# AnyLoc/Revisit-Anything

Measured on AMD Instinct MI355X. Metric: query_images_per_sec, higher is better.
Workload: dtype f32

## Files before the change

revisit-anything_amd/csrc/api.hip:

```cpp
#include <stdarg.h>
#include <stdlib.h>
#include <string.h>

#include <cmath>
#include <mutex>
#include <utility>

#include <initializer_list>

#include "ctx.h"

int segvlad_ctx::fail(int code, const char* fmt, ...) {
  va_list ap;
  va_start(ap, fmt);
  vsnprintf(err, sizeof(err), fmt, ap);
  va_end(ap);
  return code;
}

bool sv_is_device_ptr(const void* p) {
  hipPointerAttribute_t a;
  memset(&a, 0, sizeof(a));
  hipError_t e = hipPointerGetAttributes(&a, p);
  if (e != hipSuccess) {
// ... 133 lines not shown
  if (!c->profiling || c->scope_mute) return;
  t = &c->timers[name];
  if (t->used * 2 >= (int)t->ev.size()) {
    hipEvent_t a = nullptr, b = nullptr;
    (void)hipEventCreate(&a);
    (void)hipEventCreate(&b);
    t->ev.push_back(a);
    t->ev.push_back(b);
  }
  slot = t->used++;
  (void)hipEventRecord(t->ev[2 * slot], c->stream);
}
StageScope::~StageScope() {
  if (t) (void)hipEventRecord(t->ev[2 * slot + 1], ctx->stream);
}

#define CHECK_NO_OPEN_DESCRIBE(what)                                                                                        \
  if (ctx->mask_branch_on_side)                                                                                             \
  return ctx->fail(SEGVLAD_ERR_STATE, what ": a segvlad_describe_begin is open on this context (call segvlad_describe_end first)")

hipError_t sv_max_dyn_lds(const void* fn, size_t bytes) {
  static std::mutex mu;
  static std::map<std::pair<int, const void*>, size_t> done;
  int dev = 0;
  hipError_t e = hipGetDevice(&dev);
  if (e != hipSuccess) return e;
  std::lock_guard<std::mutex> lk(mu);
  auto it = done.find({dev, fn});
  if (it != done.end() && it->second >= bytes) return hipSuccess;
  e = hipFuncSetAttribute(fn, hipFuncAttributeMaxDynamicSharedMemorySize, (int)bytes);
  if (e == hipSuccess) done[{dev, fn}] = bytes;
  return e;
}

extern "C" {

int segvlad_version(void) { return 300; }

int segvlad_create(segvlad_ctx** out, int device_id) {
  if (!out) return SEGVLAD_ERR_ARG;
  *out = nullptr;
  int ndev = 0;
  if (hipGetDeviceCount(&ndev) != hipSuccess || device_id < 0 || device_id >= ndev) return SEGVLAD_ERR_HIP;
  if (hipSetDevice(device_id) != hipSuccess) return SEGVLAD_ERR_HIP;
  segvlad_ctx* c = new (std::nothrow) segvlad_ctx();
  if (!c) return SEGVLAD_ERR_NOMEM;
  c->device = device_id;
  static const char* const env_keys[][2] = {{"SEGVLAD_KNN_FILTER", "knn_filter"},   {"SEGVLAD_F16_CFG", "f16_cfg"},
                                            {"SEGVLAD_F16_GM", "f16_gm"},           {"SEGVLAD_X3_TILE", "x3_tile"},
                                            {"SEGVLAD_X3_GM", "x3_gm"},             {"SEGVLAD_SEARCH_STATS", "search_stats"},
                                            {"SEGVLAD_ASSIGN_NARROW", "assign_narrow"}, {"SEGVLAD_DEBUG_SEARCH", "debug_search"},
                                            {"SEGVLAD_AGG_KPB", "agg_kpb"},
                                            {"SEGVLAD_KNN_HEURISTIC", "knn_heuristic"}, {"SEGVLAD_PCA_PATH", "pca_path"},
                                            {"SEGVLAD_COVER_ROWS", "cover_rows"}};
  for (auto& kv : env_keys)
    if (const char* v = getenv(kv[0])) (void)segvlad_set_option(c, kv[1], v);
#define SV_TAG_P(n) c->n.tag = #n; c->n.fixed = true;
#define SV_TAG_S(n) c->n.tag = #n;
  SV_PERSISTENT_BUFS(SV_TAG_P)
  SV_SCRATCH_BUFS(SV_TAG_S)
#undef SV_TAG_P
#undef SV_TAG_S
  if (const char* v = getenv("SEGVLAD_GUARD")) {
    if (v[0] && v[0] != '0') {
      c->guard = true;
      c->for_each_buf([](DevBuf& b) { b.guard = true; });
    }
  }
  if (const char* v = getenv("SEGVLAD_RCCL_LIB")) snprintf(sv_rccl_lib_override, sizeof(sv_rccl_lib_override), "%s", v);
  if (getenv("SEGVLAD_KNN_FP32")) (void)segvlad_set_option(c, "knn_filter", "fp32");
  if (getenv("SEGVLAD_PCA_FP32")) (void)segvlad_set_option(c, "pca_arith", "fp32");
  c->err[0] = 0;
  *out = c;
  return SEGVLAD_OK;
}

int segvlad_set_option(segvlad_ctx* ctx, const char* key, const char* value) {
  if (!ctx) return SEGVLAD_ERR_ARG;
  if (!key || !value) return ctx->fail(SEGVLAD_ERR_ARG, "set_option: null key/value");
  SvOptions& o = ctx->opt;
  auto as_int = [&](int* dst) -> int {
    char* end = nullptr;
    const long v = strtol(value, &end, 10);
    if (end == value || *end) return ctx->fail(SEGVLAD_ERR_ARG, "set_option(%s): '%s' is not an integer", key, value);
    *dst = (int)v;
    return SEGVLAD_OK;
  };
  if (!strcmp(key, "knn_filter")) {
    if (!strcmp(value, "auto")) o.knn_filter = 0;
    else if (!strcmp(value, "f16")) o.knn_filter = 1;
    else if (!strcmp(value, "bf16x3")) o.knn_filter = 2;
    else if (!strcmp(value, "fp32")) o.knn_filter = 3;
    else return ctx->fail(SEGVLAD_ERR_ARG, "set_option(knn_filter): want auto|f16|bf16x3|fp32, got '%s'", value);
    return SEGVLAD_OK;
  }
  if (!strcmp(key, "pca_arith")) {
    if (!strcmp(value, "auto") || !strcmp(value, "f16x3")) o.pca_fp32 = 0;
    else if (!strcmp(value, "fp32")) o.pca_fp32 = 1;
    else return ctx->fail(SEGVLAD_ERR_ARG, "set_option(pca_arith): want auto|f16x3|fp32, got '%s'", value);
    return SEGVLAD_OK;
  }
  if (!strcmp(key, "pca_path")) {
    if (!strcmp(value, "auto")) o.pca_path = 0;
    else if (!strcmp(value, "planes")) o.pca_path = 1;
    else if (!strcmp(value, "project")) o.pca_path = 2;
    else return ctx->fail(SEGVLAD_ERR_ARG, "set_option(pca_path): want auto|planes|project, got '%s'", value);
    return SEGVLAD_OK;
  }
  auto as_dev = [&](int* dst, std::initializer_list<int> product_values, std::initializer_list<int> probe_values = {}) -> int {
    int v = *dst;
    SV_TRY(as_int(&v));
    bool ok = false;
    for (int a : product_values) ok = ok || a == v;
#ifdef SEGVLAD_ABLATIONS
    for (int a : probe_values) ok = ok || a == v;
#else
    (void)probe_values;
#endif
    if (!ok)
      return ctx->fail(SEGVLAD_ERR_ARG, "set_option(%s=%d): a development switch -- this library holds the default kernels only "
                       "(SEGVLAD_BUILD_ABLATIONS=1 builds lib/libsegvlad_hip_abl.so with the probes of csrc/segvlad_dev.h)", key, v);
    *dst = v;
    return SEGVLAD_OK;
  };
  if (!strcmp(key, "f16_cfg")) return as_dev(&o.f16_cfg, {-1, 250, 300, 62, 63}, {93, 94, 95});
  if (!strcmp(key, "f16_gm")) return as_int(&o.f16_gm);
  if (!strcmp(key, "f16_walk")) return as_int(&o.f16_walk);
  if (!strcmp(key, "f16_deep_cfg")) return as_dev(&o.f16_deep_cfg, {-1, 4, 5});
  if (!strcmp(key, "f16_buf")) return as_dev(&o.f16_buf, {-1, 0});
  if (!strcmp(key, "tnk_gram")) return as_int(&o.tnk_gram);
  if (!strcmp(key, "tnk_fork")) return as_int(&o.tnk_fork);
  if (!strcmp(key, "x3_tile")) return as_int(&o.x3_tile);
  if (!strcmp(key, "x3_gm")) return as_int(&o.x3_gm);
  if (!strcmp(key, "search_stats")) return as_int(&o.search_stats);
  if (!strcmp(key, "knn_heuristic")) return as_int(&o.knn_heuristic);
  if (!strcmp(key, "assign_narrow")) return as_int(&o.assign_narrow);
  if (!strcmp(key, "agg_kpb")) return as_int(&o.agg_kpb);
  if (!strcmp(key, "pj_nw")) return as_int(&o.pj_nw);
  if (!strcmp(key, "pj_f16")) return as_int(&o.pj_f16);
  if (!strcmp(key, "cover_rows")) return as_int(&o.cover_rows);
  if (!strcmp(key, "small_plan")) return as_int(&o.small_plan);
  if (!strcmp(key, "small_tail")) return as_int(&o.small_tail);
  if (!strcmp(key, "small_head")) return as_int(&o.small_head);
  if (!strcmp(key, "batch_l0_f16")) return as_int(&o.batch_l0_f16);
  if (!strcmp(key, "level_carry")) return as_int(&o.level_carry);
  if (!strcmp(key, "f16_persist_wgs")) return as_int(&o.f16_persist_wgs);
  if (!strcmp(key, "debug_small_tail")) return as_int(&o.debug_small_tail);
  if (!strcmp(key, "refine_group")) return as_int(&o.refine_group);
  if (!strcmp(key, "query_group")) return as_int(&o.query_group);
  if (!strcmp(key, "debug_search")) return as_int(&o.debug_search);
  if (!strcmp(key, "debug_fail_search")) return as_int(&o.debug_fail_search);
  if (!strcmp(key, "guard_undersize")) {
    if (!ctx->guard) return ctx->fail(SEGVLAD_ERR_STATE, "set_option(guard_undersize): the context was not created under SEGVLAD_GUARD=1");
    const char* colon = strchr(value, ':');
    bool found = false;
    ctx->for_each_buf([&](DevBuf& b) {
      if (!colon) b.shrink = 0;
      else if (strlen(b.tag) == (size_t)(colon - value) && !strncmp(b.tag, value, (size_t)(colon - value))) {
        b.shrink = atoi(colon + 1);
        found = true;
      }
    });
    if (colon && !found) return ctx->fail(SEGVLAD_ERR_ARG, "set_option(guard_undersize): no buffer named like '%s'", value);
    return SEGVLAD_OK;
  }
  return ctx->fail(SEGVLAD_ERR_ARG, "set_option: unknown key '%s'", key);
}

int segvlad_destroy(segvlad_ctx* ctx) {
  if (!ctx) return SEGVLAD_OK;
  (void)hipSetDevice(ctx->device);
  (void)hipStreamSynchronize(ctx->stream);
  sv_comm_release(ctx);
  if (ctx->side) {
    (void)hipStreamSynchronize(ctx->side);
    (void)hipStreamDestroy(ctx->side);
    (void)hipEventDestroy(ctx->ev_fork);
    (void)hipEventDestroy(ctx->ev_join);
  }
  if (ctx->h_pin) {
    (void)hipHostFree(ctx->h_pin);
    (void)hipEventDestroy(ctx->ev_scalars);
  }
  if (ctx->h_desc) (void)hipHostFree(ctx->h_desc);
  if (ctx->ev_desc) (void)hipEventDestroy(ctx->ev_desc);
  ctx->for_each_buf([](DevBuf& b) { b.release(); });
  for (auto& kv : ctx->timers)
    for (hipEvent_t e : kv.second.ev)
      if (e) (void)hipEventDestroy(e);
  delete ctx;
  return SEGVLAD_OK;
}

// ... 987 lines not shown
```

revisit-anything_amd/csrc/ctx.h:

```cpp
#pragma once
#include <hip/hip_runtime.h>
#include <stdint.h>
#include <stdio.h>
#include <string.h>

#include <map>
#include <string>
#include <vector>

#include "../../include/segvlad.h"

#define SV_HIP(expr)                                                                              \
  do {                                                                                            \
    hipError_t _e = (expr);                                                                       \
    if (_e != hipSuccess) {                                                                       \
      return ctx->fail(SEGVLAD_ERR_HIP, "%s failed: %s (%s:%d)", #expr, hipGetErrorString(_e),    \
                       __FILE__, __LINE__);                                                       \
    }                                                                                             \
  } while (0)

#define SV_TRY(expr)          \
  do {                        \
    int _r = (expr);          \
    if (_r != SEGVLAD_OK) return _r; \
// ... 42 lines not shown
    size_t want = bytes + bytes / 8 + 256;
    hipError_t e = hipMalloc(&p, want);
    if (e != hipSuccess) return e;
    cap = want;
    return hipSuccess;
  }
  hipError_t reserve_guarded(size_t bytes);
  size_t fence_off() const { return fixed ? cap : ((req > (size_t)shrink ? req - (size_t)shrink : 0) + 3) & ~(size_t)3; }
  void release() {
    if (raw) (void)hipFree(raw);
    else if (p) (void)hipFree(p);
    raw = nullptr;
    p = nullptr;
    cap = 0;
    req = 0;
  }
  template <class T>
  T* as() { return reinterpret_cast<T*>(p); }
};

struct StageTimer {
  std::vector<hipEvent_t> ev;
  int used = 0;
  int launches = 0;
};

struct SvOptions {
  int knn_filter = 0;
  int pca_fp32 = 0;
  int f16_cfg = -1;
  int f16_gm = -1;
  int f16_walk = -1;
  int f16_persist_wgs = 32;
  int f16_deep_cfg = -1;
  int f16_buf = -1;
  int tnk_gram = 1;
  int tnk_fork = 1;
  int x3_tile = 0;
  int x3_gm = -1;
  int search_stats = 0;
  int knn_heuristic = 1;
  int assign_narrow = 0;
  int agg_kpb = 4;
  int debug_fail_search = 0;
  int debug_search = 0;
  int debug_small_tail = 0;
  int batch_l0_f16 = 1;
  int level_carry = 1;
  int small_head = 1;
  int small_tail = 1;
  int small_plan = 1;
  int pj_f16 = 1;
  int pj_nw = 8;
  int refine_group = 1;
  int query_group = 0;
  int pca_path = 0;
  int cover_rows = 1;
};

constexpr int SV_F16_KBLOCK = 1024;
inline int sv_f16_kblock(const SvOptions& o, int d) {
  if (o.f16_cfg == 300) return SV_F16_KBLOCK;
  return (o.f16_cfg < 0 && d >= 4096) ? SV_F16_KBLOCK : 0;
}
constexpr int SV_F16_KFLUSH = 64;
int sv_f16_eps_kblock(const SvOptions& o, int d);
inline bool sv_f16_bias_possible(const SvOptions& o, int64_t nq) { return nq > 128 && (o.f16_cfg < 0 || o.f16_cfg == 250 || o.f16_cfg == 300); }
enum class F16Kernel {
  None, BatchDefault, BatchComplement, BatchSmall, BatchUnbiased, BatchUnbiasedSmall, DeepFlush, DeepFlushComplement, DeepBlockedBuf, DeepBlocked,
  DeepBlockedBufComplement, DeepBlockedComplement, DeepUnbiased, OneImage64, OneImage128,
#ifdef SEGVLAD_ABLATIONS
  ProbePhases, ProbeNoEpilogue, ProbeNoEpilogueNoDma,
#endif
};
struct F16Choice {
  F16Kernel kernel;
  const char* why;
};
F16Choice sv_choose_f16_kernel(const SvOptions& o, bool bias_ok, int M, int64_t n_rows, int d, int b_stride, int skip);
inline float sv_f16_c_eps(int d, int kb, float bias_mult) {
  const float acc = kb > 0 ? (2.f * (float)kb + (float)((d + kb - 1) / kb) + 1.f) / 16777216.f : 2.f * (float)d / 16777216.f;
  return 2.5f * (1.f / 1024.f + 1.f / 4194304.f + bias_mult * acc);
}

struct SvSearchStats {
  int64_t levels = 0;
  int64_t filter = 0;
  int64_t n_fallback = 0;
  int64_t cand_max = 0;
  int64_t cand_sum = 0;
  int64_t refine_max = 0;
  int64_t refine_sum = 0;
  int64_t n_queries = 0;
  int64_t n_redo = 0;
  int64_t n_refine2 = 0;
  int64_t grp_groups = 0;
  int64_t grp_union_sum = 0;
  int64_t carry_rows = 0;
};

struct segvlad_ctx {
  int device = 0;
  hipStream_t stream = nullptr;
  hipStream_t side = nullptr;
  hipEvent_t ev_fork = nullptr, ev_join = nullptr;
  uint32_t* h_pin = nullptr;
// ... 281 lines not shown
```

revisit-anything_amd/csrc/project_kernels.hip:

```cpp
#include "ctx.h"

typedef float f32x16 __attribute__((ext_vector_type(16)));
#define MFMA32(a, b, c) __builtin_amdgcn_mfma_f32_32x32x2f32((a), (b), (c), 0, 0, 0)
__device__ __forceinline__ int pj_frag_row(int r, int kk) { return (r & 3) + 8 * (r >> 2) + 4 * kk; }

__global__ __launch_bounds__(1024) void group_plan_kernel(const int32_t* __restrict__ cov_cnt, int B, int K,
                                                          int32_t* __restrict__ rowbase, int32_t* __restrict__ tile_group,
                                                          int max_tiles) {
  __shared__ int32_t part[1024], base[257];
  const int nsl = 1024 / K;
  const int k = threadIdx.x % K, c = threadIdx.x / K;
  const int per = (B + nsl - 1) / nsl, b0 = c * per, b1 = min(B, b0 + per);
  const bool act = c < nsl;
  for (int t = threadIdx.x; t < max_tiles; t += blockDim.x) tile_group[t] = -1;
  int sum = 0;
  if (act)
    for (int b = b0; b < b1; ++b) sum += cov_cnt[(size_t)b * K + k];
  part[threadIdx.x] = act ? sum : 0;
  __syncthreads();
  if ((int)threadIdx.x < K) {
    int run = 0;
    for (int q = 0; q < nsl; ++q) {
      const int v = part[q * K + threadIdx.x];
      part[q * K + threadIdx.x] = run;
// ... 1 lines not shown
    }
    base[threadIdx.x + 1] = (run + 255) & ~255;
  }
  __syncthreads();
  if (threadIdx.x == 0) {
    base[0] = 0;
    for (int q = 0; q < K; ++q) base[q + 1] += base[q];
  }
  __syncthreads();
  if (act) {
    int run = base[k] + part[threadIdx.x];
    for (int b = b0; b < b1; ++b) {
      rowbase[(size_t)b * K + k] = run;
      run += cov_cnt[(size_t)b * K + k];
    }
  }
  __syncthreads();
  if ((int)threadIdx.x < K)
    for (int t = base[threadIdx.x] >> 8; t < (base[threadIdx.x + 1] >> 8) && t < max_tiles; ++t) tile_group[t] = threadIdx.x;
}

int sv_launch_group_plan(segvlad_ctx* ctx, const int32_t* cov_cnt, int B, int K, int32_t* rowbase, int32_t* tile_group,
                         int max_tiles) {
  if (K > 256) return ctx->fail(SEGVLAD_ERR_LIMIT, "group_plan: K=%d > 256", K);
  hipLaunchKernelGGL(group_plan_kernel, dim3(1), dim3(1024), 0, ctx->stream, cov_cnt, B, K, rowbase, tile_group, max_tiles);
  SV_HIP(hipGetLastError());
  return SEGVLAD_OK;
}

__global__ __launch_bounds__(256) void project_consts_kernel(const float* __restrict__ comps, const float* __restrict__ mean,
                                                             int P, int64_t KD, float* __restrict__ wmu) {
  const int p = blockIdx.x;
  const float* w = comps + (size_t)p * KD;
  double acc = 0.0;
  for (int64_t j = threadIdx.x; j < KD; j += 256) acc += (double)w[j] * (double)mean[j];
  __shared__ double red[256];
  red[threadIdx.x] = acc;
  __syncthreads();
  for (int o = 128; o > 0; o >>= 1) {
    if ((int)threadIdx.x < o) red[threadIdx.x] += red[threadIdx.x + o];
    __syncthreads();
  }
  if (threadIdx.x == 0) wmu[p] = (float)red[0];
}

int sv_launch_project_consts(segvlad_ctx* ctx, const float* comps, const float* mean, int P, int64_t KD, float* wmu) {
  hipLaunchKernelGGL(project_consts_kernel, dim3(P), dim3(256), 0, ctx->stream, comps, mean, P, KD, wmu);
  SV_HIP(hipGetLastError());
  return SEGVLAD_OK;
}

constexpr int PJ_T = 32;

template <int NW, bool F16 = false>
__global__ __launch_bounds__(64 * NW) void project_aggregate_kernel(const float* __restrict__ Z, const float* __restrict__ wmu,
                                                                const float* __restrict__ bn, const float* __restrict__ gscale,
                                                                const uint64_t* __restrict__ colmask,
                                                                const int32_t* __restrict__ lab_off,
                                                                const int32_t* __restrict__ rowbase,
                                                                const int32_t* __restrict__ phys,
                                                                const int32_t* __restrict__ seg_off, int N, int K, int P, int SC,
                                                                int maxt, const float* __restrict__ col_scale,
                                                                float* __restrict__ Y, float zscale) {
  extern __shared__ __attribute__((aligned(16))) unsigned char smem[];
  typedef _Float16 f16x8 __attribute__((ext_vector_type(8)));
  static_assert(!F16 || NW == 8, "16-bit tile sums: the 8-wave workgroup");
  const int KS = K + 1 + (K & 1);
  float* ag = reinterpret_cast<float*>(smem);
  constexpr int NC = 32 * NW, NT_ = 64 * NW, C4W = NC / 4;
  float* zt = ag + 64 * KS;
  uint64_t* mk = reinterpret_cast<uint64_t*>(zt + 2 * PJ_T * NC);
  int32_t* tl_k = reinterpret_cast<int32_t*>(mk + 2 * PJ_T);
  int32_t* tl_j = tl_k + maxt;
  int32_t* tl_z = tl_j + maxt;
  int32_t* tl_n = tl_z + maxt;
  int32_t* phl = tl_n + maxt + K + 1;
  uint4* af = reinterpret_cast<uint4*>((reinterpret_cast<uintptr_t>(phl + N) + 15) & ~(uintptr_t)15);
  __shared__ int s_tiles;
  const int b = blockIdx.y, p0 = blockIdx.x * NC;
  const int tid = threadIdx.x, w = tid >> 6, l = tid & 63, i = l & 31, kk = l >> 5;
  const int s0 = seg_off[b], S = seg_off[b + 1] - s0;
  const int SCb = (S + 63) >> 6;
  const int32_t* lo = lab_off + (size_t)b * (K + 1);
  const int pcol = p0 + 32 * w + i;
  int32_t* tl_pre = tl_n + maxt;
  int my_o0 = 0, my_n = 0, my_g0 = 0;
  if (tid < K) {
    my_o0 = lo[tid];
    my_n = lo[tid + 1] - my_o0;
    my_g0 = rowbase[(size_t)b * K + tid];
    tl_pre[tid + 1] = (my_n + PJ_T - 1) / PJ_T;
  }
  for (int j = tid; j < N; j += NT_) phl[j] = phys[(size_t)b * N + j];
  __syncthreads();
  if (tid == 0) {
    int run = 0;
    tl_pre[0] = 0;
    for (int k = 0; k < K; ++k) {
      run += tl_pre[k + 1];
      tl_pre[k + 1] = run;
    }
    s_tiles = run < maxt ? run : maxt;
  }
  __syncthreads();
  if (tid < K) {
    int t = tl_pre[tid];
    for (int j0 = 0; j0 < my_n && t < maxt; j0 += PJ_T, ++t) {
      tl_k[t] = tid;
      tl_j[t] = my_o0 + j0;
      tl_z[t] = my_g0;
      tl_n[t] = min(PJ_T, my_n - j0);
    }
  }
  __syncthreads();
  const int tiles = s_tiles;

  for (int sc = 0; sc < SCb; ++sc) {
    const int Sc = min(64, S - 64 * sc);
    __syncthreads();
    for (int idx = tid; idx < 64 * K; idx += NT_) {
      const int s = idx / K, k = idx - s * K;
      float a = 0.f;
      if (s < Sc) {
        const float nrm = bn[(size_t)(s0 + 64 * sc + s) * K + k];
        a = nrm > 1e-12f ? gscale[s0 + 64 * sc + s] / nrm : 0.f;
      }
      if (F16) ag[k * 64 + s] = a;
      else ag[s * KS + k] = a;
    }
    f32x16 acc[2];
// ... 73 lines not shown
      _Pragma("unroll") for (int ks = 0; ks < 2; ++ks) {                                                        \
        if (ks == 1 && nt_ <= 16) break;                                                                        \
        f16x8 hh, ll;                                                                                           \
        _Pragma("unroll") for (int e = 0; e < 8; ++e) {                                                         \
          const float v = ztc[(size_t)(16 * ks + e) * NC] * zscale;                                             \
          hh[e] = (_Float16)v;                                                                                  \
          ll[e] = (_Float16)(v - (float)hh[e]);                                                                 \
        }                                                                                                       \
        const uint4 a0u = afc[(2 * ks) * 64];                                                                   \
        const f16x8 a0 = __builtin_bit_cast(f16x8, a0u);                                                        \
        if (ks == 0) {                                                                                          \
          f32x16 zero_;                                                                                         \
          _Pragma("unroll") for (int r = 0; r < 16; ++r) zero_[r] = 0.f;                                        \
          ta0 = __builtin_amdgcn_mfma_f32_32x32x16_f16(a0, ll, zero_, 0, 0, 0);                                 \
        } else {                                                                                                \
          ta0 = __builtin_amdgcn_mfma_f32_32x32x16_f16(a0, ll, ta0, 0, 0, 0);                                   \
        }                                                                                                       \
        ta0 = __builtin_amdgcn_mfma_f32_32x32x16_f16(a0, hh, ta0, 0, 0, 0);                                     \
        if (two) {                                                                                              \
          const uint4 a1u = afc[(2 * ks + 1) * 64];                                                             \
          const f16x8 a1 = __builtin_bit_cast(f16x8, a1u);                                                      \
          if (ks == 0) {                                                                                        \
            f32x16 zero_;                                                                                       \
            _Pragma("unroll") for (int r = 0; r < 16; ++r) zero_[r] = 0.f;                                      \
            ta1 = __builtin_amdgcn_mfma_f32_32x32x16_f16(a1, ll, zero_, 0, 0, 0);                               \
          } else {                                                                                              \
            ta1 = __builtin_amdgcn_mfma_f32_32x32x16_f16(a1, ll, ta1, 0, 0, 0);                                 \
          }                                                                                                     \
          ta1 = __builtin_amdgcn_mfma_f32_32x32x16_f16(a1, hh, ta1, 0, 0, 0);                                   \
        }                                                                                                       \
      }                                                                                                         \
       \
      const float* agk = ag + k_ * 64 + 4 * kk;                                                                 \
      _Pragma("unroll") for (int q = 0; q < 4; ++q) {                                                           \
        const float4 w0 = *reinterpret_cast<const float4*>(agk + 8 * q);                                        \
        acc[0][4 * q + 0] = fmaf(w0.x, ta0[4 * q + 0], acc[0][4 * q + 0]);                                      \
        acc[0][4 * q + 1] = fmaf(w0.y, ta0[4 * q + 1], acc[0][4 * q + 1]);                                      \
        acc[0][4 * q + 2] = fmaf(w0.z, ta0[4 * q + 2], acc[0][4 * q + 2]);                                      \
        acc[0][4 * q + 3] = fmaf(w0.w, ta0[4 * q + 3], acc[0][4 * q + 3]);                                      \
        if (two) {                                                                                              \
          const float4 w1 = *reinterpret_cast<const float4*>(agk + 32 + 8 * q);                                 \
          acc[1][4 * q + 0] = fmaf(w1.x, ta1[4 * q + 0], acc[1][4 * q + 0]);                                    \
          acc[1][4 * q + 1] = fmaf(w1.y, ta1[4 * q + 1], acc[1][4 * q + 1]);                                    \
          acc[1][4 * q + 2] = fmaf(w1.z, ta1[4 * q + 2], acc[1][4 * q + 2]);                                    \
          acc[1][4 * q + 3] = fmaf(w1.w, ta1[4 * q + 3], acc[1][4 * q + 3]);                                    \
        }                                                                                                       \
      }                                                                                                         \
    } while (0)
#define SV_PJ_MULX(t_)                                                                                          \
    do {                                                                                                        \
      if constexpr (F16) SV_PJ_MUL16(t_);                                                                       \
      else SV_PJ_MUL(t_);                                                                                       \
    } while (0)
    if (tiles > 0) {
      SV_PJ_FETCH(va, ma, 0);
      SV_PJ_FETCH_F(fa, 0);
      SV_PJ_STASH(va, ma, 0);
      SV_PJ_STASH_F(fa, 0);
    }
    if (tiles > 1) {
      SV_PJ_FETCH(va, ma, 1);
      SV_PJ_FETCH_F(fa, 1);
    }
    __syncthreads();
    for (int t = 0; t < tiles; t += 2) {
      if (t + 2 < tiles) {
        SV_PJ_FETCH(vb, mb, t + 2);
        SV_PJ_FETCH_F(fb, t + 2);
      }
      SV_PJ_MULX(t);
      if (t + 1 < tiles) {
        SV_PJ_STASH(va, ma, 1);
        SV_PJ_STASH_F(fa, 1);
      }
      __syncthreads();
      if (t + 1 >= tiles) break;
      if (t + 3 < tiles) {
        SV_PJ_FETCH(va, ma, t + 3);
        SV_PJ_FETCH_F(fa, t + 3);
      }
      SV_PJ_MULX(t + 1);
      if (t + 2 < tiles) {
        SV_PJ_STASH(vb, mb, 0);
        SV_PJ_STASH_F(fb, 0);
      }
      __syncthreads();
    }
#undef SV_PJ_MULX
#undef SV_PJ_MUL16
#undef SV_PJ_STASH_F
#undef SV_PJ_FETCH_F
#undef SV_PJ_MUL
#undef SV_PJ_STASH
#undef SV_PJ_FETCH
    if (pcol < P) {
      const float cs = col_scale ? col_scale[pcol] : 1.f, mu = wmu[pcol];
#pragma unroll
      for (int mt = 0; mt < 2; ++mt) {
        if (mt == 1 && !two) break;
#pragma unroll
        for (int r = 0; r < 16; ++r) {
          const int s = 32 * mt + pj_frag_row(r, kk);
          if (s < Sc) Y[(size_t)(s0 + 64 * sc + s) * P + pcol] = ((F16 ? acc[mt][r] * (1.f / zscale) : acc[mt][r]) - mu) * cs;
        }
      }
    }
  }
}

int sv_launch_project_aggregate(segvlad_ctx* ctx, const float* Z, const float* wmu, const float* block_norms, const float* gscale,
                                const uint64_t* colmask, const int32_t* lab_off, const int32_t* rowbase, const int32_t* phys,
                                const int32_t* seg_off_dev, int B, int N, int K, int P, int SC, int S_max, const float* col_scale,
                                float* Y, float zscale) {
  if (B <= 0 || S_max <= 0) return SEGVLAD_OK;
  if (P % 4) return ctx->fail(SEGVLAD_ERR_ARG, "project_aggregate: P=%d must be a multiple of 4", P);
  const int maxt = K + (N + PJ_T - 1) / PJ_T;
  const int nw = ctx->opt.pj_nw == 4 ? 4 : 8;
  if (K > 64 * nw) return ctx->fail(SEGVLAD_ERR_LIMIT, "project_aggregate: K=%d clusters need %d threads", K, K);
  const bool f16 = zscale > 0.f && nw == 8 && ctx->opt.pj_f16 != 0;
  const size_t lds = (size_t)64 * (K + 1 + (K & 1)) * 4 + (size_t)2 * PJ_T * 32 * nw * 4 + (size_t)2 * PJ_T * 8 + (size_t)4 * maxt * 4 +
                     (size_t)(K + 1) * 4 + (size_t)N * 4 + (f16 ? 16 + 2 * 256 * 16 : 0);
  if (lds > 160 * 1024)
    return ctx->fail(SEGVLAD_ERR_LIMIT, "project_aggregate: K=%d, N=%d need %zu B of LDS", K, N, lds);
  const void* fn = f16 ? reinterpret_cast<const void*>(project_aggregate_kernel<8, true>)
                       : nw == 8 ? reinterpret_cast<const void*>(project_aggregate_kernel<8>) : reinterpret_cast<const void*>(project_aggregate_kernel<4>);
  if (lds > 64 * 1024) SV_HIP(sv_max_dyn_lds(fn, (size_t)lds));
  const dim3 grid((P + 32 * nw - 1) / (32 * nw), B), block(64 * nw);
  if (f16)
    hipLaunchKernelGGL((project_aggregate_kernel<8, true>), grid, block, lds, ctx->stream, Z, wmu, block_norms, gscale, colmask, lab_off,
                       rowbase, phys, seg_off_dev, N, K, P, SC, maxt, col_scale, Y, zscale);
  else if (nw == 8)
    hipLaunchKernelGGL(project_aggregate_kernel<8>, grid, block, lds, ctx->stream, Z, wmu, block_norms, gscale, colmask, lab_off, rowbase,
                       phys, seg_off_dev, N, K, P, SC, maxt, col_scale, Y, 0.f);
  else
    hipLaunchKernelGGL(project_aggregate_kernel<4>, grid, block, lds, ctx->stream, Z, wmu, block_norms, gscale, colmask, lab_off, rowbase,
                       phys, seg_off_dev, N, K, P, SC, maxt, col_scale, Y, 0.f);
  SV_HIP(hipGetLastError());
  return SEGVLAD_OK;
}
```

revisit-anything_amd/csrc/vlad_kernels.hip:

```cpp
#include <stdio.h>
#include <stdlib.h>

#include "ctx.h"

typedef float f32x16 __attribute__((ext_vector_type(16)));

#define MFMA32(a, b, c) __builtin_amdgcn_mfma_f32_32x32x2f32((a), (b), (c), 0, 0, 0)

template <int CTRL>
__device__ __forceinline__ float dpp_f32(float x) {
  return __int_as_float(__builtin_amdgcn_update_dpp(0, __float_as_int(x), CTRL, 0xf, 0xf, true));
}

__device__ __forceinline__ int frag_row(int r, int kk) { return (r & 3) + 8 * (r >> 2) + 4 * kk; }

__global__ void vocab_norm_kernel(const float* __restrict__ C, int K, int D, float* __restrict__ inv) {
  const int k = blockIdx.x;
  float s = 0.f;
  for (int d = threadIdx.x; d < D; d += blockDim.x) {
    float v = C[(size_t)k * D + d];
    s = fmaf(v, v, s);
  }
  __shared__ float red[256];
  red[threadIdx.x] = s;
// ... 537 lines not shown
  _Pragma("unroll") for (int j = 0; j < 4; ++j) {                                     \
    const int d_ = lr + 8 * j;                                                        \
    float* q = tile + (buf) * (DC * TS) + d_ * TS + ((4 * lq + rot(d_)) & 127);       \
    *reinterpret_cast<float4*>(q) = V[j];                                             \
  }
  SV_LOAD_CHUNK(va, 0)
  SV_PARK_CHUNK(va, 0)
  if (1 < nch) { SV_LOAD_CHUNK(va, 1) }
  __syncthreads();
#define SV_ASSIGN_STEP(c, VNEXT, VFREE)                                               \
  {                                                                                   \
    if ((c) + 2 < nch) { SV_LOAD_CHUNK(VFREE, (c) + 2) }                              \
    assign_wide_chunk<NT>(tile + ((c) & 1) * (DC * TS), bt, Xt, b, N, D, t0, tid, w, l, i, kk, (c), acc, ss);  \
    if ((c) + 1 < nch) { SV_PARK_CHUNK(VNEXT, ((c) + 1) & 1) }                        \
    __syncthreads();                                                                  \
  }
  for (int c = 0; c < nch; c += 2) {
    SV_ASSIGN_STEP(c, va, vb)
    if (c + 1 < nch) SV_ASSIGN_STEP(c + 1, vb, va)
  }
#undef SV_ASSIGN_STEP
#undef SV_LOAD_CHUNK
#undef SV_PARK_CHUNK
  constexpr int KP = NT * 32;
  float* sc = tile;
  ss += __shfl_xor(ss, 32);
  if (kk == 0) ssum[32 * w + i] = ss;
#pragma unroll
  for (int n = 0; n < NT; ++n)
#pragma unroll
    for (int r = 0; r < 16; ++r) sc[(32 * w + frag_row(r, kk)) * (KP + 1) + n * 32 + i] = acc[n][r];
  __syncthreads();
  if (tid < 128 && t0 + tid < N) {
    const float rn = 1.0f / fmaxf(sqrtf(ssum[tid]), 1e-12f);
    float best = -INFINITY, second = -INFINITY;
    int bi = 0;
    for (int k = 0; k < K; ++k) {
      const float sv = sc[tid * (KP + 1) + k];
      if (sv > best) {
        second = best;
        best = sv;
        bi = k;
      } else if (sv > second) {
        second = sv;
      }
    }
    const size_t o = (size_t)b * N + t0 + tid;
    labels[o] = (uint8_t)bi;
    rnorm[o] = rn;
    if (gap) gap[o] = (K > 1) ? (best - second) * rn : INFINITY;
  }
}

int sv_launch_assign(segvlad_ctx* ctx, const float* tokens, int B, int N, float* xt, uint8_t* labels, float* rnorm,
                     float* gap) {
  const int NT = ctx->Kpad / 32;
  dim3 grid((N + 63) / 64, B), block(256);
  const float* bt = ctx->vocab_bt.as<float>();
  if (NT <= 2 && ctx->D % 32 == 0 && !ctx->opt.assign_narrow) {
    const unsigned tiles_total = (unsigned)((N + 127) / 128) * (unsigned)B;
    dim3 gridw((tiles_total + 7) / 8 * 8, 1);
    if (NT == 1)
      hipLaunchKernelGGL(assign_wide_kernel<1>, gridw, block, 0, ctx->stream, tokens, N, ctx->D, ctx->K, bt, xt, labels, rnorm, gap, B);
    else
      hipLaunchKernelGGL(assign_wide_kernel<2>, gridw, block, 0, ctx->stream, tokens, N, ctx->D, ctx->K, bt, xt, labels, rnorm, gap, B);
    SV_HIP(hipGetLastError());
    return SEGVLAD_OK;
  }
  switch (NT) {
    case 1:
      hipLaunchKernelGGL(assign_kernel<1>, grid, block, 0, ctx->stream, tokens, N, ctx->D, ctx->K, bt, xt, labels, rnorm, gap);
      break;
    case 2: {
#ifdef SEGVLAD_ABLATIONS
      const char* ab = getenv("SEGVLAD_ASSIGN_ABL");
      const int a = ab ? atoi(ab) : 0;
      if (a == 1) {
        hipLaunchKernelGGL((assign_kernel<2, 1>), grid, block, 0, ctx->stream, tokens, N, ctx->D, ctx->K, bt, xt, labels, rnorm, gap);
        break;
      } else if (a == 2) {
        hipLaunchKernelGGL((assign_kernel<2, 2>), grid, block, 0, ctx->stream, tokens, N, ctx->D, ctx->K, bt, xt, labels, rnorm, gap);
        break;
      } else if (a == 3) {
        hipLaunchKernelGGL((assign_kernel<2, 3>), grid, block, 0, ctx->stream, tokens, N, ctx->D, ctx->K, bt, xt, labels, rnorm, gap);
        break;
      }
#endif
      hipLaunchKernelGGL(assign_kernel<2>, grid, block, 0, ctx->stream, tokens, N, ctx->D, ctx->K, bt, xt, labels, rnorm, gap);
      break;
    }
    case 4:
      hipLaunchKernelGGL(assign_kernel<4>, grid, block, 0, ctx->stream, tokens, N, ctx->D, ctx->K, bt, xt, labels, rnorm, gap);
      break;
    default:
      return ctx->fail(SEGVLAD_ERR_LIMIT, "K=%d: supported cluster counts are 1..64 and 97..128 (Kpad in {32,64,128})", ctx->K);
  }
  SV_HIP(hipGetLastError());
  return SEGVLAD_OK;
}

__global__ __launch_bounds__(256) void prep_kernel(const uint8_t* __restrict__ labels, const uint64_t* __restrict__ inc,
                                                   const int32_t* __restrict__ seg_off,
                                                   const int64_t* __restrict__ adj_off, const uint8_t* __restrict__ adj,
                                                   int N, int K, int S_max, int SC, uint64_t* __restrict__ colmask,
                                                   float* __restrict__ gscale, int32_t* __restrict__ tok_order,
                                                   int32_t* __restrict__ lab_off, const float* __restrict__ rnorm,
                                                   float* __restrict__ rn_sorted, int stage, int ord_n,
                                                   int32_t* __restrict__ phys, int32_t* __restrict__ cov_cnt, int cover) {
  extern __shared__ __attribute__((aligned(16))) unsigned char smem[];
  const int b = blockIdx.x;
  const int nw = (N + 63) >> 6;
  const int s0 = seg_off[b], S = seg_off[b + 1] - s0;
  uint64_t* inc2 = reinterpret_cast<uint64_t*>(smem);
  uint64_t* lbits = inc2 + (size_t)S_max * nw;
// ... 858 lines not shown
```

Baseline: 8680.

## Add register-staged software pipelining to assign and project-aggregate kernels

Adds new scheduled variants of the assign kernel and the project-aggregate kernel. Both prefetch the next tiles into registers two steps ahead and park them into double-buffered LDS after the MFMA work, so global loads overlap compute. The assign variant can also double-buffer the vocabulary slice. The variants are on by default through a new describe_sched option, and launches now go through hipLaunchKernel with an argument array. This uses more registers and LDS, which may lower occupancy.

```diff
diff --git a/revisit-anything_amd/csrc/api.hip b/revisit-anything_amd/csrc/api.hip
--- a/revisit-anything_amd/csrc/api.hip
+++ b/revisit-anything_amd/csrc/api.hip
@@ -209,7 +209,7 @@
                                             {"SEGVLAD_ASSIGN_NARROW", "assign_narrow"}, {"SEGVLAD_DEBUG_SEARCH", "debug_search"},
                                             {"SEGVLAD_AGG_KPB", "agg_kpb"},
                                             {"SEGVLAD_KNN_HEURISTIC", "knn_heuristic"}, {"SEGVLAD_PCA_PATH", "pca_path"},
-                                            {"SEGVLAD_COVER_ROWS", "cover_rows"}};
+                                            {"SEGVLAD_COVER_ROWS", "cover_rows"},   {"SEGVLAD_DESCRIBE_SCHED", "describe_sched"}};
   for (auto& kv : env_keys)
     if (const char* v = getenv(kv[0])) (void)segvlad_set_option(c, kv[1], v);
 #define SV_TAG_P(n) c->n.tag = #n; c->n.fixed = true;
@@ -296,6 +296,7 @@
   if (!strcmp(key, "pj_nw")) return as_int(&o.pj_nw);
   if (!strcmp(key, "pj_f16")) return as_int(&o.pj_f16);
   if (!strcmp(key, "cover_rows")) return as_int(&o.cover_rows);
+  if (!strcmp(key, "describe_sched")) return as_int(&o.describe_sched);
   if (!strcmp(key, "small_plan")) return as_int(&o.small_plan);
   if (!strcmp(key, "small_tail")) return as_int(&o.small_tail);
   if (!strcmp(key, "small_head")) return as_int(&o.small_head);
diff --git a/revisit-anything_amd/csrc/ctx.h b/revisit-anything_amd/csrc/ctx.h
--- a/revisit-anything_amd/csrc/ctx.h
+++ b/revisit-anything_amd/csrc/ctx.h
@@ -118,6 +118,7 @@
   int small_plan = 1;
   int pj_f16 = 1;
   int pj_nw = 8;
+  int describe_sched = 1;
   int refine_group = 1;
   int query_group = 0;
   int pca_path = 0;
diff --git a/revisit-anything_amd/csrc/project_kernels.hip b/revisit-anything_amd/csrc/project_kernels.hip
--- a/revisit-anything_amd/csrc/project_kernels.hip
+++ b/revisit-anything_amd/csrc/project_kernels.hip
@@ -77,7 +77,7 @@
 
 constexpr int PJ_T = 32;
 
-template <int NW, bool F16 = false>
+template <int NW, bool F16 = false, bool SCHED = false>
 __global__ __launch_bounds__(64 * NW) void project_aggregate_kernel(const float* __restrict__ Z, const float* __restrict__ wmu,
                                                                 const float* __restrict__ bn, const float* __restrict__ gscale,
                                                                 const uint64_t* __restrict__ colmask,
@@ -100,7 +100,8 @@
   int32_t* tl_z = tl_j + maxt;
   int32_t* tl_n = tl_z + maxt;
   int32_t* phl = tl_n + maxt + K + 1;
-  uint4* af = reinterpret_cast<uint4*>((reinterpret_cast<uintptr_t>(phl + N) + 15) & ~(uintptr_t)15);
+  uint4* af = SCHED ? reinterpret_cast<uint4*>(smem + ((static_cast<size_t>(reinterpret_cast<unsigned char*>(phl + N) - smem) + 15) & ~(size_t)15))
+                    : reinterpret_cast<uint4*>((reinterpret_cast<uintptr_t>(phl + N) + 15) & ~(uintptr_t)15);
   __shared__ int s_tiles;
   const int b = blockIdx.y, p0 = blockIdx.x * NC;
   const int tid = threadIdx.x, w = tid >> 6, l = tid & 63, i = l & 31, kk = l >> 5;
@@ -280,6 +281,75 @@
       if constexpr (F16) SV_PJ_MUL16(t_);                                                                       \
       else SV_PJ_MUL(t_);                                                                                       \
     } while (0)
+#define SV_PJ_FETCH_S(V, KM, M, R, NTV, t_)                                                                      \
+    do {                                                                                                        \
+      const int nt_ = tl_n[t_], j_ = tl_j[t_];                                                                  \
+      const float* src_ = Z + (size_t)tl_z[t_] * P;                                                             \
+      const int32_t* ph_ = phl + j_;                                                                            \
+      NTV = nt_;                                                                                                \
+      KM = 0u;                                                                                                  \
+      _Pragma("unroll") for (int q = 0; q < 4; ++q) {                                                           \
+        const int idx4 = tid + NT_ * q, row = idx4 / C4W, c4 = idx4 % C4W;                                      \
+        const int pr_ = row < nt_ ? ph_[row] : -1;                                                              \
+        const bool ok_ = pr_ >= 0 && p0 + 4 * c4 < P;                                                           \
+        KM |= ok_ ? (1u << q) : 0u;                                                                             \
+        V[q] = *reinterpret_cast<const float4*>(ok_ ? src_ + (size_t)pr_ * P + p0 + 4 * c4 : Z);                \
+      }                                                                                                         \
+      if constexpr (F16) {                                                                                      \
+        const int j0_ = 16 * ((tid >> 7) & 1) + 8 * ((tid & 63) >> 5);                                          \
+        const uint32_t* mrow_ = reinterpret_cast<const uint32_t*>(colmask + ((size_t)b * N + j_) * SC + sc) + ((tid >> 6) & 1); \
+        _Pragma("unroll") for (int e = 0; e < 8; ++e) R[e] = mrow_[(size_t)min(j0_ + e, nt_ - 1) * SC * 2];     \
+      } else {                                                                                                  \
+        M = colmask[((size_t)b * N + j_ + min(tid & (PJ_T - 1), nt_ - 1)) * SC + sc];                           \
+      }                                                                                                         \
+    } while (0)
+#define SV_PJ_STASH_S(V, KM, M, R, NTV, buf_)                                                                    \
+    do {                                                                                                        \
+      _Pragma("unroll") for (int q = 0; q < 4; ++q) {                                                           \
+        const int idx4 = tid + NT_ * q, row = idx4 / C4W, c4 = idx4 % C4W;                                      \
+        *reinterpret_cast<float4*>(zt + (size_t)(buf_) * PJ_T * NC + row * NC + 4 * c4) =                       \
+            ((KM >> q) & 1u) ? V[q] : make_float4(0.f, 0.f, 0.f, 0.f);                                          \
+      }                                                                                                         \
+      if constexpr (F16) {    \
+        const int s5_ = tid & 31, j0_ = 16 * ((tid >> 7) & 1) + 8 * ((tid & 63) >> 5);                          \
+        uint32_t d_[4];                                                                                         \
+        _Pragma("unroll") for (int q = 0; q < 4; ++q) {                                                         \
+          const bool b0_ = j0_ + 2 * q < NTV && ((R[2 * q] >> s5_) & 1u);                                       \
+          const bool b1_ = j0_ + 2 * q + 1 < NTV && ((R[2 * q + 1] >> s5_) & 1u);                               \
+          d_[q] = (b0_ ? 0x3C00u : 0u) | (b1_ ? 0x3C000000u : 0u);                                              \
+        }                                                                                                       \
+        if (tid < 256) af[(buf_) * 256 + tid] = make_uint4(d_[0], d_[1], d_[2], d_[3]);                         \
+      } else {                                                                                                  \
+        if (tid < PJ_T) mk[(buf_) * PJ_T + tid] = tid < NTV ? M : 0ull;                                         \
+      }                                                                                                         \
+    } while (0)
+#define SV_PJ_STEP(t_, VN, KN, MN, RN, NN, VF, KF, MF, RF, NF, MORE)                                             \
+    {                                                                                                           \
+      if (MORE || (t_) + 2 < tiles) SV_PJ_FETCH_S(VF, KF, MF, RF, NF, (t_) + 2);                                \
+      SV_PJ_MULX(t_);                                                                                           \
+      if (MORE || (t_) + 1 < tiles) SV_PJ_STASH_S(VN, KN, MN, RN, NN, ((t_) + 1) & 1);                          \
+      __syncthreads();                                                                                          \
+    }
+    if constexpr (SCHED) {
+      unsigned ka = 0u, kb = 0u;
+      int na = 0, nb = 0;
+      uint32_t ra[8], rb[8];
+      if (tiles > 0) {
+        SV_PJ_FETCH_S(va, ka, ma, ra, na, 0);
+        SV_PJ_STASH_S(va, ka, ma, ra, na, 0);
+      }
+      if (tiles > 1) SV_PJ_FETCH_S(va, ka, ma, ra, na, 1);
+      __syncthreads();
+      int t = 0;
+      for (; t + 3 < tiles; t += 2) {
+        SV_PJ_STEP(t, va, ka, ma, ra, na, vb, kb, mb, rb, nb, true)
+        SV_PJ_STEP(t + 1, vb, kb, mb, rb, nb, va, ka, ma, ra, na, true)
+      }
+      for (; t < tiles; t += 2) {
+        SV_PJ_STEP(t, va, ka, ma, ra, na, vb, kb, mb, rb, nb, false)
+        if (t + 1 < tiles) SV_PJ_STEP(t + 1, vb, kb, mb, rb, nb, va, ka, ma, ra, na, false)
+      }
+    } else {
     if (tiles > 0) {
       SV_PJ_FETCH(va, ma, 0);
       SV_PJ_FETCH_F(fa, 0);
@@ -314,6 +384,10 @@
       }
       __syncthreads();
     }
+    }
+#undef SV_PJ_STEP
+#undef SV_PJ_STASH_S
+#undef SV_PJ_FETCH_S
 #undef SV_PJ_MULX
 #undef SV_PJ_MUL16
 #undef SV_PJ_STASH_F
@@ -333,6 +407,7 @@
         }
       }
     }
+    if constexpr (SCHED) __builtin_amdgcn_s_waitcnt(0x0F70);
   }
 }
 
@@ -350,19 +425,20 @@
                      (size_t)(K + 1) * 4 + (size_t)N * 4 + (f16 ? 16 + 2 * 256 * 16 : 0);
   if (lds > 160 * 1024)
     return ctx->fail(SEGVLAD_ERR_LIMIT, "project_aggregate: K=%d, N=%d need %zu B of LDS", K, N, lds);
-  const void* fn = f16 ? reinterpret_cast<const void*>(project_aggregate_kernel<8, true>)
-                       : nw == 8 ? reinterpret_cast<const void*>(project_aggregate_kernel<8>) : reinterpret_cast<const void*>(project_aggregate_kernel<4>);
+  const bool sched = ctx->opt.describe_sched != 0;
+  const void* fn = sched ? (f16       ? reinterpret_cast<const void*>(project_aggregate_kernel<8, true, true>)
+                            : nw == 8 ? reinterpret_cast<const void*>(project_aggregate_kernel<8, false, true>)
+                                      : reinterpret_cast<const void*>(project_aggregate_kernel<4, false, true>))
+                         : (f16       ? reinterpret_cast<const void*>(project_aggregate_kernel<8, true>)
+                            : nw == 8 ? reinterpret_cast<const void*>(project_aggregate_kernel<8>)
+                                      : reinterpret_cast<const void*>(project_aggregate_kernel<4>));
   if (lds > 64 * 1024) SV_HIP(sv_max_dyn_lds(fn, (size_t)lds));
   const dim3 grid((P + 32 * nw - 1) / (32 * nw), B), block(64 * nw);
-  if (f16)
-    hipLaunchKernelGGL((project_aggregate_kernel<8, true>), grid, block, lds, ctx->stream, Z, wmu, block_norms, gscale, colmask, lab_off,
-                       rowbase, phys, seg_off_dev, N, K, P, SC, maxt, col_scale, Y, zscale);
-  else if (nw == 8)
-    hipLaunchKernelGGL(project_aggregate_kernel<8>, grid, block, lds, ctx->stream, Z, wmu, block_norms, gscale, colmask, lab_off, rowbase,
-                       phys, seg_off_dev, N, K, P, SC, maxt, col_scale, Y, 0.f);
-  else
-    hipLaunchKernelGGL(project_aggregate_kernel<4>, grid, block, lds, ctx->stream, Z, wmu, block_norms, gscale, colmask, lab_off, rowbase,
-                       phys, seg_off_dev, N, K, P, SC, maxt, col_scale, Y, 0.f);
+  const float zs = f16 ? zscale : 0.f;
+  void* args[] = {(void*)&Z,    (void*)&wmu,     (void*)&block_norms, (void*)&gscale, (void*)&colmask, (void*)&lab_off, (void*)&rowbase,
+                  (void*)&phys, (void*)&seg_off_dev, (void*)&N,       (void*)&K,      (void*)&P,       (void*)&SC,      (void*)&maxt,
+                  (void*)&col_scale, (void*)&Y,  (void*)&zs};
+  SV_HIP(hipLaunchKernel(fn, grid, block, args, lds, ctx->stream));
   SV_HIP(hipGetLastError());
   return SEGVLAD_OK;
 }
diff --git a/revisit-anything_amd/csrc/vlad_kernels.hip b/revisit-anything_amd/csrc/vlad_kernels.hip
--- a/revisit-anything_amd/csrc/vlad_kernels.hip
+++ b/revisit-anything_amd/csrc/vlad_kernels.hip
@@ -613,6 +613,143 @@
   }
 }
 
+template <int NT, int NB>
+__global__ __launch_bounds__(256, NB == 1 ? 4 : 3) void assign_sched_kernel(const float* __restrict__ T, int N, int D, int K,
+                                                           const float* __restrict__ bt, float* __restrict__ Xt,
+                                                           uint8_t* __restrict__ labels, float* __restrict__ rnorm,
+                                                           float* __restrict__ gap, int B) {
+  constexpr int DC = 32, TS = 128, BL = (DC / 2) * NT * 64;
+  constexpr int KP = NT * 32;
+  auto rot = [](int d) { return 8 * (d >> 2) + 32 * (d & 1); };
+  __shared__ __attribute__((aligned(16))) float lds[2 * DC * TS + NB * BL];
+  static_assert(128 * (KP + 1) + 128 <= 2 * DC * TS + NB * BL, "the scores and the squared norms reuse the tiles");
+  float* tile = lds;
+  float* bl = lds + 2 * DC * TS;
+  const int gx = (N + 127) / 128;
+  const int per = (int)((gridDim.x + 7) / 8);
+  const int logical = (int)(blockIdx.x & 7) * per + (int)(blockIdx.x >> 3);
+  if (logical >= gx * B) return;
+  const int b = logical / gx, t0 = (logical - b * gx) * 128;
+  const int tid = threadIdx.x, w = tid >> 6, l = tid & 63, i = l & 31, kk = l >> 5;
+  const float* Tb = T + (size_t)b * D * N;
+  const int lr = tid >> 5, lq = tid & 31;
+  const int tl0 = t0 + 4 * lq;
+  const int col = min(tl0, N - 4);
+  const int sh = tl0 - col;
+  const bool edge = t0 + 128 > N;
+  f32x16 acc[NT];
+#pragma unroll
+  for (int n = 0; n < NT; ++n)
+#pragma unroll
+    for (int r = 0; r < 16; ++r) acc[n][r] = 0.f;
+  float ss = 0.f;
+  const int nch = D / DC;
+  float4 va[4], vb[4], bq0, bq1 = make_float4(0.f, 0.f, 0.f, 0.f);
+#define SV_LOAD_B(c)                                                                  \
+  {                                                                                   \
+    bq0 = *reinterpret_cast<const float4*>(bt + (size_t)(c) * BL + 4 * tid);          \
+    if (NT == 2) bq1 = *reinterpret_cast<const float4*>(bt + (size_t)(c) * BL + 4 * (tid + 256)); \
+  }
+#define SV_PARK_B(buf)                                                                \
+  {                                                                                   \
+    *reinterpret_cast<float4*>(bl + (buf) * BL + 4 * tid) = bq0;                      \
+    if (NT == 2) *reinterpret_cast<float4*>(bl + (buf) * BL + 4 * (tid + 256)) = bq1; \
+  }
+#define SV_LOAD_CHUNK(V, c)                                                           \
+  _Pragma("unroll") for (int j = 0; j < 4; ++j) {                                     \
+    const f32x4u u = *reinterpret_cast<const f32x4u*>(Tb + (size_t)((c) * DC + lr + 8 * j) * N + col); \
+    V[j] = make_float4(u[0], u[1], u[2], u[3]);                                       \
+  }
+#define SV_PARK_CHUNK(V, buf)                                                         \
+  _Pragma("unroll") for (int j = 0; j < 4; ++j) {                                     \
+    const int d_ = lr + 8 * j;                                                        \
+    float* q = tile + (buf) * (DC * TS) + d_ * TS + ((4 * lq + rot(d_)) & 127);       \
+    float4 v = V[j];                                                                  \
+    if (edge)                                                                         \
+      v = sh == 0 ? v : sh == 1 ? make_float4(v.y, v.z, v.w, 0.f) : sh == 2 ? make_float4(v.z, v.w, 0.f, 0.f) \
+                  : sh == 3 ? make_float4(v.w, 0.f, 0.f, 0.f) : make_float4(0.f, 0.f, 0.f, 0.f); \
+    *reinterpret_cast<float4*>(q) = v;                                                \
+  }
+  SV_LOAD_B(0)
+  SV_LOAD_CHUNK(va, 0)
+  SV_PARK_B(0)
+  SV_PARK_CHUNK(va, 0)
+  if (1 < nch) { SV_LOAD_CHUNK(va, 1) }
+  __syncthreads();
+#define SV_ASSIGN_STEP(c, VNEXT, VFREE, MORE)                                         \
+  {                                                                                   \
+    const float* tl = tile + ((c) & 1) * (DC * TS);                                   \
+    const float* blc = bl + (NB == 2 ? (c) & 1 : 0) * BL + l;                         \
+    if (MORE || (c) + 1 < nch) { SV_LOAD_B((c) + 1) }                                 \
+    if (MORE || (c) + 2 < nch) { SV_LOAD_CHUNK(VFREE, (c) + 2) }                      \
+    _Pragma("unroll 8") for (int st = 0; st < DC / 2; ++st) {                         \
+      const float x = tl[(2 * st + kk) * TS + ((32 * w + i + rot(2 * st + kk)) & 127)]; \
+      ss = fmaf(x, x, ss);                                                            \
+      _Pragma("unroll") for (int n = 0; n < NT; ++n) acc[n] = MFMA32(x, blc[(st * NT + n) * 64], acc[n]); \
+    }                                                                                 \
+    if (NB == 1) __syncthreads();           \
+     \
+                                                          \
+    if (MORE || (c) + 1 < nch) {                                                      \
+      SV_PARK_B(NB == 2 ? ((c) + 1) & 1 : 0)                                          \
+      SV_PARK_CHUNK(VNEXT, ((c) + 1) & 1)                                             \
+    }                                                                                 \
+    _Pragma("unroll") for (int it = 0; it < 4; ++it) {                                \
+      const int idx = it * 256 + tid;                                                 \
+      const int tok = idx >> 3, c4 = idx & 7;                                         \
+      if (t0 + tok < N) {                                                             \
+        const float* q = tl + (4 * c4) * TS;                                          \
+        const int t_a = (tok + 8 * c4) & 127, t_b = (tok + 8 * c4 + 32) & 127;        \
+        const float4 o = make_float4(q[t_a], q[TS + t_b], q[2 * TS + t_a], q[3 * TS + t_b]); \
+        *reinterpret_cast<float4*>(Xt + ((size_t)b * N + t0 + tok) * D + (c) * DC + 4 * c4) = o; \
+      }                                                                               \
+    }                                                                                 \
+    __syncthreads();                                                                  \
+  }
+  int c = 0;
+  for (; c + 3 < nch; c += 2) {
+    SV_ASSIGN_STEP(c, va, vb, true)
+    SV_ASSIGN_STEP(c + 1, vb, va, true)
+  }
+  for (; c < nch; c += 2) {
+    SV_ASSIGN_STEP(c, va, vb, false)
+    if (c + 1 < nch) SV_ASSIGN_STEP(c + 1, vb, va, false)
+  }
+#undef SV_ASSIGN_STEP
+#undef SV_LOAD_CHUNK
+#undef SV_PARK_CHUNK
+#undef SV_LOAD_B
+#undef SV_PARK_B
+  float* sc = lds;
+  float* ssum = sc + 128 * (KP + 1);
+  ss += __shfl_xor(ss, 32);
+  if (kk == 0) ssum[32 * w + i] = ss;
+#pragma unroll
+  for (int n = 0; n < NT; ++n)
+#pragma unroll
+    for (int r = 0; r < 16; ++r) sc[(32 * w + frag_row(r, kk)) * (KP + 1) + n * 32 + i] = acc[n][r];
+  __syncthreads();
+  if (tid < 128 && t0 + tid < N) {
+    const float rn = 1.0f / fmaxf(sqrtf(ssum[tid]), 1e-12f);
+    float best = -INFINITY, second = -INFINITY;
+    int bi = 0;
+    for (int k = 0; k < K; ++k) {
+      const float sv = sc[tid * (KP + 1) + k];
+      if (sv > best) {
+        second = best;
+        best = sv;
+        bi = k;
+      } else if (sv > second) {
+        second = sv;
+      }
+    }
+    const size_t o = (size_t)b * N + t0 + tid;
+    labels[o] = (uint8_t)bi;
+    rnorm[o] = rn;
+    if (gap) gap[o] = (K > 1) ? (best - second) * rn : INFINITY;
+  }
+}
+
 int sv_launch_assign(segvlad_ctx* ctx, const float* tokens, int B, int N, float* xt, uint8_t* labels, float* rnorm,
                      float* gap) {
   const int NT = ctx->Kpad / 32;
@@ -621,6 +758,15 @@
   if (NT <= 2 && ctx->D % 32 == 0 && !ctx->opt.assign_narrow) {
     const unsigned tiles_total = (unsigned)((N + 127) / 128) * (unsigned)B;
     dim3 gridw((tiles_total + 7) / 8 * 8, 1);
+    if (ctx->opt.describe_sched != 0 && N >= 4) {
+      const bool two = ctx->opt.describe_sched != 2;
+      const void* fn = NT == 1 ? (two ? (const void*)assign_sched_kernel<1, 2> : (const void*)assign_sched_kernel<1, 1>)
+                               : (two ? (const void*)assign_sched_kernel<2, 2> : (const void*)assign_sched_kernel<2, 1>);
+      const int K_ = ctx->K, D_ = ctx->D;
+      void* args[] = {(void*)&tokens, (void*)&N, (void*)&D_, (void*)&K_, (void*)&bt, (void*)&xt, (void*)&labels, (void*)&rnorm, (void*)&gap, (void*)&B};
+      SV_HIP(hipLaunchKernel(fn, gridw, block, args, 0, ctx->stream));
+      return SEGVLAD_OK;
+    }
     if (NT == 1)
       hipLaunchKernelGGL(assign_wide_kernel<1>, gridw, block, 0, ctx->stream, tokens, N, ctx->D, ctx->K, bt, xt, labels, rnorm, gap, B);
     else
```

Result: no change. 8760 (median of 6 runs) (+0.9%).
